# prip-lab/MSU-LatentAFIS

Hardware: AMD Instinct MI355X
Metric: latent queries/sec vs 100k rolled gallery (higher is better)
Workload: dtype f32

## Files before the change

msu-latentafis_amd/csrc/graph.hip:

```cpp
#include "afis_device.h"
#include <type_traits>
#include "atan2f_libm.h"
#include "graph_arith.h"
#include "stdsort_order.h"

namespace afis {

#define AFIS_PI 3.1415926
typedef unsigned long long u64;

#ifdef AFIS_PHASE_TIMING
__device__ u64 g_graph_phase[16];
#define GPH_INIT() u64 gph_t0 = __builtin_readcyclecounter()
#define GPH(i) do { if (threadIdx.x == 0) { const u64 t1_ = __builtin_readcyclecounter(); sm.ph[(i)] += t1_ - gph_t0; gph_t0 = t1_; } } while (0)
#define GPH_T0() const u64 gph_k0 = __builtin_readcyclecounter()
#define GPH_K(i) do { if (threadIdx.x == 0) sm.ph[(i)] += __builtin_readcyclecounter() - gph_k0; } while (0)
#define GPH_ZERO() do { if (threadIdx.x < 16) sm.ph[threadIdx.x] = 0; WSYNC(); } while (0)
#define GPH_FLUSH() do { WSYNC(); if (threadIdx.x < 16 && sm.ph[threadIdx.x]) atomicAdd(&g_graph_phase[threadIdx.x], sm.ph[threadIdx.x]); } while (0)
#else
#define GPH_INIT() do {} while (0)
#define GPH(i) do {} while (0)
#define GPH_T0() do {} while (0)
#define GPH_K(i) do {} while (0)
#define GPH_ZERO() do {} while (0)
// ... 103 lines not shown
template <class SM, int ref_tie>
__device__ __forceinline__ void sort_scores(SM& sm, int num, double thr)
{
    const int lane = threadIdx.x;
    constexpr int U = SM::U;
    uint32_t* const s_key = reinterpret_cast<uint32_t*>(sm.x.s.keys);
    uint32_t* const s_cnt = s_key + SM::N4;
    uint32_t* const s_gkey = reinterpret_cast<uint32_t*>(sm.y.cc);
    static_assert(sizeof(sm.x) >= (size_t)(SM::N4 + 128) * 4, "sort scratch exceeds the union");
    uint32_t m32[U]; int r[U];
    if (num <= 48) {
        const u64 mine = lane < num ? g_make_key(sm.b[lane], lane) : 0ull;
        if (lane < num) sm.x.s.keys[lane] = mine;
        WSYNC();
        int rr = 0;
        for (int k = 0; k < num; ++k) rr += sm.x.s.keys[k] > mine;
        if (ref_tie && num > 16) {
            int gg = 0;
            for (int k = 0; k < num; ++k) gg += (uint32_t)(sm.x.s.keys[k] >> 32) > (uint32_t)(mine >> 32);
            const bool tied = lane < num && gg != rr && !((double)sm.b[lane] < thr);
            if (__ballot(tied) != 0ull) {
                uint32_t* const k32 = reinterpret_cast<uint32_t*>(sm.x.s.keys) + 96;
                static_assert(sizeof(sm.x.s.keys) >= (96 + 48 + 48) * 4, "no room for the keys and the stack of the std::sort restatement");
                WSYNC();
                if (lane < num) { k32[lane] = (uint32_t)(mine >> 32); sm.y.os.order[lane] = (short)lane; }
                WSYNC();
                if (lane == 0) stdsort_prefix<uint16_t>(reinterpret_cast<uint16_t*>(sm.y.os.order), num, num, k32, reinterpret_cast<int*>(k32 + 48));
                WSYNC();
                return;
            }
        }
        WSYNC();
        if (lane < num) sm.y.os.order[rr] = (short)lane;
        WSYNC();
        return;
    }
    uint32_t kmin = 0xffffffffu, kmax = 0u;
#pragma unroll
    for (int u = 0; u < U; ++u) {
        const int t = lane + 64 * u;
        m32[u] = t < num ? g_ord_f32(sm.b[t]) : 0u;
        if (t < num) { s_key[t] = m32[u]; kmin = min(kmin, m32[u]); kmax = max(kmax, m32[u]); }
    }
#pragma unroll
    for (int off = 32; off >= 1; off >>= 1) { kmin = min(kmin, (uint32_t)__shfl_xor((int)kmin, off)); kmax = max(kmax, (uint32_t)__shfl_xor((int)kmax, off)); }
    const uint32_t span = kmax - kmin;
    const int sh = max(0, 26 - __clz((int)(span | 1u)));
    int bin[U];
#pragma unroll
    for (int u = 0; u < U; ++u) bin[u] = (int)((m32[u] - kmin) >> sh) & 63;
    s_cnt[lane] = 0u;
    WSYNC();
#pragma unroll
    for (int u = 0; u < U; ++u) if (lane + 64 * u < num) atomicAdd(&s_cnt[bin[u]], 1u);
    WSYNC();
    {
        const int own = (int)s_cnt[lane];
        int suf = own;
#pragma unroll
        for (int off = 1; off < 64; off <<= 1) { const int v = __shfl_down(suf, off); if (lane + off < 64) suf += v; }
        WSYNC();
        s_cnt[lane] = (uint32_t)(suf - own); s_cnt[64 + lane] = (uint32_t)(suf - own);
    }
    WSYNC();
#pragma unroll
    for (int u = 0; u < U; ++u) if (lane + 64 * u < num) s_gkey[atomicAdd(&s_cnt[bin[u]], 1u)] = m32[u];
    WSYNC();
    int rsum = 0;
#pragma unroll
    for (int u = 0; u < U; ++u) {
        r[u] = 0;
        if (lane + 64 * u < num) {
            const int lo = (int)s_cnt[64 + bin[u]], hi = (int)s_cnt[bin[u]];
            int c = lo;
            for (int k = lo; k < hi; ++k) c += s_gkey[k] > m32[u];
            r[u] = c; rsum += c;
        }
    }
    if (g_wave_sum(rsum) != num * (num - 1) / 2) {
        u64 mine[U];
        int gg[U];
#pragma unroll
        for (int u = 0; u < U; ++u) { const int t = lane + 64 * u; mine[u] = t < num ? ((u64)m32[u] << 32) | (uint32_t)(~(uint32_t)t) : 0ull; r[u] = 0; gg[u] = 0; }
        for (int k = 0; k < num; ++k) {
            const u64 kk = ((u64)s_key[k] << 32) | (uint32_t)(~(uint32_t)k);
#pragma unroll
            for (int u = 0; u < U; ++u) { r[u] += kk > mine[u]; gg[u] += s_key[k] > m32[u]; }
        }
        if (ref_tie) {
            bool tied = false;
#pragma unroll
            for (int u = 0; u < U; ++u) { const int t = lane + 64 * u; tied |= t < num && gg[u] != r[u] && !((double)sm.b[t] < thr); }
            if (__ballot(tied) != 0ull) {
                WSYNC();
#pragma unroll
                for (int u = 0; u < U; ++u) { const int t = lane + 64 * u; if (t < num) sm.y.os.order[t] = (short)t; }
                WSYNC();
                if (lane == 0) stdsort_prefix<uint16_t>(reinterpret_cast<uint16_t*>(sm.y.os.order), num, num, s_key, reinterpret_cast<int*>(s_cnt));
                WSYNC();
                return;
            }
        }
    }
    WSYNC();
#pragma unroll
    for (int u = 0; u < U; ++u) { const int t = lane + 64 * u; if (t < num) sm.y.os.order[r[u]] = (short)t; }
    WSYNC();
}

template <class SM, class Compat>
__device__ int greedy(SM& sm, int num, double thr, Compat compatible)
{
    const int lane = threadIdx.x;
    constexpr int U = SM::U;
    int idx[U], li[U], ri[U];
    bool alive[U];
#pragma unroll
    for (int u = 0; u < U; ++u) {
        const int p = lane + 64 * u;
        idx[u] = 0; li[u] = -1; ri[u] = -1; alive[u] = false;
        if (p < num) {
            idx[u] = sm.y.os.order[p];
            li[u] = l_row<SM>(sm.li[idx[u]]); ri[u] = r_pt<SM>(sm.ri[idx[u]]);
            alive[u] = !((double)sm.b[idx[u]] < thr);
        }
    }
    int nsel = 0;
    for (;;) {
        int first = -1, cidx = 0, cli = 0, cri = 0;
#pragma unroll
        for (int u = 0; u < U; ++u) {
            const u64 m = __ballot(alive[u]);
            if (first < 0 && m) {
                const int fl = __ffsll((long long)m) - 1;
                first = 64 * u + fl;
                cidx = __shfl(idx[u], fl); cli = __shfl(li[u], fl); cri = __shfl(ri[u], fl);
            }
        }
        if (first < 0) break;
        if (lane == 0) sm.y.os.sel[nsel] = (short)cidx;
        ++nsel;
#pragma unroll
        for (int u = 0; u < U; ++u) {
            if (alive[u]) {
                const int p = lane + 64 * u;
                if (p == first || li[u] == cli || ri[u] == cri || !compatible(cidx, idx[u])) alive[u] = false;
            }
        }
    }
    WSYNC();
    return nsel;
}

template <class SM>
__device__ void compact(SM& sm, int n)
{
    const int lane = threadIdx.x;
    float sim[SM::U]; short li[SM::U], ri[SM::U]; int2 xy[SM::U];
#pragma unroll
    for (int u = 0; u < SM::U; ++u) {
        const int t = lane + 64 * u;
        sim[u] = 0.0f;
        if (t < n) { const int s = sm.y.os.sel[t]; if constexpr (SM::OWN_SIM) sim[u] = sm.simv[s]; li[u] = sm.li[s]; ri[u] = sm.ri[s]; xy[u] = sm.xy[s]; }
    }
    WSYNC();
#pragma unroll
    for (int u = 0; u < SM::U; ++u) {
        const int t = lane + 64 * u;
        if (t < n) { if constexpr (SM::OWN_SIM) sm.simv[t] = sim[u]; sm.li[t] = li[u]; sm.ri[t] = ri[u]; sm.xy[t] = xy[u]; }
    }
    WSYNC();
}

template <class SM>
__device__ __forceinline__ float seq_sum(const SM& sm, int num)
{
    float sum = 0.0f;
    const float4* c4 = reinterpret_cast<const float4*>(sm.y.cc);
#pragma unroll 4
    for (int k = 0; k < (num + 3) / 4; ++k) { const float4 v = c4[k]; sum += v.x; sum += v.y; sum += v.z; sum += v.w; }
    return sum;
}

template <bool LOOKUP>
__device__ __forceinline__ bool pair_dist(const Pt& a, const Pt& o, const float* __restrict__ table, float& dist)
{
    float d1, d2; bool ok = true;
    if (LOOKUP) {
        const int dx1 = abs(a.lx - o.lx), dx2 = abs(a.rx - o.rx), dy1 = abs(a.ly - o.ly), dy2 = abs(a.ry - o.ry);
        ok = !((dx1 >= kDistN) | (dx2 >= kDistN) | (dy1 >= kDistN) | (dy2 >= kDistN));
        d1 = sqrt_rn_pos((float)(256 * (dx1 * dx1 + dy1 * dy1)));
        d2 = sqrt_rn_pos((float)(256 * (dx2 * dx2 + dy2 * dy2)));
        (void)table;
    } else {
        const float dx1 = (float)(a.lx - o.lx), dx2 = (float)(a.rx - o.rx), dy1 = (float)(a.ly - o.ly), dy2 = (float)(a.ry - o.ry);
        const float p = dx1 * dx1, q = dy1 * dy1, r = dx2 * dx2, s = dy2 * dy2;
        d1 = sqrt_rn_pos(p + q);
        d2 = sqrt_rn_pos(r + s);
    }
    dist = fabsf(d1 - d2);
    return ok;
}
template <bool LOOKUP>
__device__ __forceinline__ bool pair_compatible(const Pt& a, const Pt& o, const float* __restrict__ table)
{
    float s1, s2; bool ok = true;
    if (LOOKUP) {
        const int dx1 = abs(a.lx - o.lx), dx2 = abs(a.rx - o.rx), dy1 = abs(a.ly - o.ly), dy2 = abs(a.ry - o.ry);
        ok = !((dx1 >= kDistN) | (dx2 >= kDistN) | (dy1 >= kDistN) | (dy2 >= kDistN));
        s1 = (float)(256 * (dx1 * dx1 + dy1 * dy1)); s2 = (float)(256 * (dx2 * dx2 + dy2 * dy2));
    } else {
        const float dx1 = (float)(a.lx - o.lx), dx2 = (float)(a.rx - o.rx), dy1 = (float)(a.ly - o.ly), dy2 = (float)(a.ry - o.ry);
        const float p = dx1 * dx1, q = dy1 * dy1, r = dx2 * dx2, s = dy2 * dy2;
        s1 = p + q; s2 = r + s;
    }
    const float d1 = __builtin_amdgcn_sqrtf(s1), d2 = __builtin_amdgcn_sqrtf(s2);
    const float dist = fabsf(d1 - d2);
    const float slack = fmaxf(d1, d2) * 4.76837158e-7f;
    if (fabsf(dist - 30.0f) > slack) return ok && dist < 30.0f;
    float exact;
    pair_dist<LOOKUP>(a, o, table, exact);
    return ok && exact < 30.0f;
}
template <bool RANGE_TEST>
__device__ __forceinline__ bool tex_pair_dist(int2 a, int2 o, float& dist)
{
    float n1, n2;
    pair_n(a, o, n1, n2);
    dist = 16.0f * fabsf(sqrt_rn_int(n1) - sqrt_rn_int(n2));
    return RANGE_TEST ? tex_in_range(a, o) : true;
}
template <bool RANGE_TEST>
__device__ __forceinline__ bool tex_pair_compatible(int2 a, int2 o)
{
    float n1, n2;
    pair_n(a, o, n1, n2);
    const bool ok = RANGE_TEST ? tex_in_range(a, o) : true;
    return pair_compatible_n<true>(n1, n2) && ok;
}

__device__ __forceinline__ float minu_pair_dist(int2 a, int2 o)
{
    float n1, n2;
    pair_n(a, o, n1, n2);
    return fabsf(sqrt_rn_int(n1) - sqrt_rn_int(n2));
}
__device__ __forceinline__ bool minu_pair_compatible(int2 a, int2 o)
{
    float n1, n2;
    pair_n(a, o, n1, n2);
    return pair_compatible_n<false>(n1, n2);
}

__device__ __forceinline__ float h_of_x(float x)
{
    const float q0 = x * 0.04f;
    const float r = fmaf(-q0, 25.0f, x);
    const float h = fmaf(r, 0.04f, q0);
    return __builtin_amdgcn_fmed3f(h, 0.0f, 1.0f);
}
__device__ __forceinline__ float h_value(float dist)
{
    const float x = 30.0f - dist;
    const float q0 = x * 0.04f;
    const float r = fmaf(-q0, 25.0f, x);
    const float h = fmaf(r, 0.04f, q0);
    return __builtin_amdgcn_fmed3f(h, 0.0f, 1.0f);
}

template <class SM, bool LOOKUP, int ITERS, int MODE, int REF_TIE>
__device__ int dist_filter(SM& sm, int num, const float* __restrict__ table, const float* __restrict__ ext, SlabBuf slab)
{
    constexpr bool fast = MODE > 0;
    constexpr bool range_test = MODE == 1;
    auto compat_fast = [](int2 a, int2 o) -> bool { if (LOOKUP) return tex_pair_compatible<range_test>(a, o); return minu_pair_compatible(a, o); };
    auto dist_fast = [](int2 a, int2 o) -> float { float d; if (LOOKUP) { tex_pair_dist<range_test>(a, o, d); return d; } return minu_pair_dist(a, o); };
    constexpr int U = SM::U, W = SM::W, NMAX = SM::NMAX;
    [[maybe_unused]] constexpr int PH = LOOKUP ? 8 : 0;
    GPH_INIT();
    const int lane = threadIdx.x;
    for (int i = lane; i < num * W; i += 64) sm.hb[i / W][i % W] = 0u;
    int2 me[U];
#pragma unroll
    for (int u = 0; u < U; ++u) {
        const int t = lane + 64 * u;
        if (t < SM::N4) { sm.b[t] = t < num ? list_sim(sm, ext, t) : 0.0f; sm.y.cc[t] = 0.0f; }
        me[u] = t < num ? sm.xy[t] : make_int2(0, 0);
    }
    WSYNC();
    const int half = num >> 1;
    const bool even = !(num & 1);
    uint32_t* const hb0 = &sm.hb[0][0];
    auto pair = [&](int2 own, int t, int k, int2 other) {
        if (fast ? compat_fast(own, other) : pair_compatible<LOOKUP>(unpack_xy(own), unpack_xy(other), table)) {
            atomicOr(hb0 + (t * W + (k >> 5)), 1u << (k & 31));
            atomicOr(hb0 + (__umul24(k, W) + (t >> 5)), 1u << (t & 31));
        }
    };
    const int tail0 = num & ~63, R = num - tail0;
    const bool grouped = R > 0 && R <= 32;
    const int n_wide = grouped ? tail0 : num;
    uint32_t kb[U];
    const uint32_t num8 = (uint32_t)num * 8u;
#pragma unroll
    for (int u = 0; u < U; ++u) { const int t = lane + 64 * u; kb[u] = t < num ? (uint32_t)t * 8u : 0u; }
#ifndef AFIS_PAIR_UNROLL
// ... 59 lines not shown
    const int n_blk = (n_wide + 63) >> 6;
    if (n_blk >= U) pair_loop(std::integral_constant<int, U>{});
    else if (U > 1 && n_blk == U - 1) pair_loop(std::integral_constant<int, (U > 1 ? U - 1 : 1)>{});
    else if (n_blk > 0) pair_loop(std::integral_constant<int, U>{});
    if (grouped) {
        const int sh = R <= 8 ? 3 : R <= 16 ? 4 : 5, RG = 1 << sh, dstep = 64 >> sh;
        const int r = lane & (RG - 1), t = tail0 + r;
        const bool row = r < R;
        const int2 own = row ? sm.xy[t] : make_int2(0, 0);
        int d = 1 + (lane >> sh);
        int k = t + d; k = k >= num ? k - num : k;
        for (int d0 = 1; d0 <= half; d0 += dstep) {
            if (row && d <= half && !(d == half && even && t >= half)) pair(own, t, k, sm.xy[k]);
            d += dstep; k += dstep; k = k >= num ? k - num : k;
        }
    }
    WSYNC();
    GPH(PH + 0);
    int myrow[U], trip[U], rlen[U];
    const int Wn = (num + 31) / 32;
    {
        int cnt[U];
#pragma unroll
        for (int u = 0; u < U; ++u) {
            const int t = lane + 64 * u;
            int c = -1;
            if (t < num) {
                c = 0; for (int w = 0; w < Wn; ++w) c += __popc(sm.hb[t][w]);
                sm.y.os.sel[t] = (short)c;
                c = min(c >> 2, 15);
            }
            cnt[u] = c;
        }
        int base = 0;
        for (int bk = 15; bk >= 0; --bk) {
#pragma unroll
            for (int u = 0; u < U; ++u) {
                const bool in = cnt[u] == bk;
                const u64 m = __ballot(in);
                if (in) sm.y.os.order[base + g_lane_prefix(m)] = (short)(lane + 64 * u);
                base += __popcll(m);
            }
        }
        WSYNC();
#pragma unroll
        for (int u = 0; u < U; ++u) {
            const int p = lane + 64 * u;
            myrow[u] = p < num ? (int)sm.y.os.order[p] : -1;
            rlen[u] = myrow[u] >= 0 ? (int)sm.y.os.sel[myrow[u]] : 0;
            trip[u] = g_wave_max(rlen[u]);
        }
        WSYNC();
        for (int t = num + lane; t < SM::N4; t += 64) sm.y.cc[t] = 0.0f;
    }
    int2 mine[U];
#pragma unroll
    for (int u = 0; u < U; ++u) mine[u] = myrow[u] >= 0 ? sm.xy[myrow[u]] : make_int2(0, 0);
    constexpr bool kFlat = NMAX > 128;
    constexpr int kSlabN = kFlat ? kTexSlabSteps : kMinuSlabSteps;
    static_assert(kSlabN % 4 == 0, "the read loop takes blocks of four steps");
    static_assert((size_t)U * kSlabN * 64 * 5 == (kFlat ? kTexSlabWgBytes : kMinuSlabWgBytes), "slab layout and the size the host allocates differ");
    constexpr int kSlabBlk = kSlabN / 4;
    constexpr uint32_t kSlabIdx0 = (uint32_t)U * kSlabN * 64 * 4;
    const uint32_t lane16 = (uint32_t)lane * 16u, lane4 = (uint32_t)lane * 4u;
    auto put_block = [&](int e, const float (&h)[4], uint32_t k4) {
        __builtin_amdgcn_raw_buffer_store_b128(v4u{__float_as_uint(h[0]), __float_as_uint(h[1]), __float_as_uint(h[2]), __float_as_uint(h[3])}, slab, lane16, e * 1024, 0);
        __builtin_amdgcn_raw_buffer_store_b32(k4, slab, lane4, (int)kSlabIdx0 + e * 256, 0);
    };
    auto get_block = [&](int e, v4u& h, uint32_t& k4) {
        h = __builtin_amdgcn_raw_buffer_load_b128(slab, lane16, e * 1024, 0);
        k4 = __builtin_amdgcn_raw_buffer_load_b32(slab, lane4, (int)kSlabIdx0 + e * 256, 0);
    };
    int cur_w[U]; uint32_t cur_bits[U];
#pragma unroll
    for (int u = 0; u < U; ++u) { cur_w[u] = 0; cur_bits[u] = 0u; }
    auto value = [&](int2 own, int k) -> float {
        float dist;
        if (fast && LOOKUP) {
            float n1, n2;
            pair_n(own, sm.xy[k], n1, n2);
            return h_of_x(fmaf(-16.0f, fabsf(sqrt_rn_int(n1) - sqrt_rn_int(n2)), 30.0f));
        }
        if (fast) dist = dist_fast(own, sm.xy[k]);
        else pair_dist<LOOKUP>(unpack_xy(own), unpack_xy(sm.xy[k]), table, dist);
        return h_value(dist);
    };
    for (int it = 0; it < ITERS; ++it) {
#pragma unroll
        for (int u = 0; u < U; ++u) {
            const int t = myrow[u];
            const uint32_t* hrow = sm.hb[t >= 0 ? t : 0];
            float acc = 0.0f;
            if (it == 0) {
                if (t >= 0) {
                    int w = 0;
                    uint32_t bits = hrow[0];
                    for (int n0 = 0; n0 < trip[u]; n0 += 4) {
                        if (n0 == kSlabN) { cur_w[u] = w; cur_bits[u] = bits; }
                        float h4[4] = {0.0f, 0.0f, 0.0f, 0.0f};
                        uint32_t k4 = 0u;
#pragma unroll
                        for (int j = 0; j < 4; ++j) {
                            if (n0 + j < trip[u]) {
                                while (bits == 0u && w + 1 < Wn) { ++w; bits = hrow[w]; }
                                const bool have = bits != 0u;
                                const int k = (w * 32 + __ffs(bits) - 1) & 255;
                                bits &= bits - 1;
                                const float h = value(mine[u], k);
                                h4[j] = h; k4 |= (uint32_t)k << (8 * j);
                                const float p = h * sm.b[k];
                                acc += have ? p : 0.0f;
                            }
                        }
                        if (n0 < kSlabN) put_block(u * kSlabBlk + (n0 >> 2), h4, k4);
                    }
                }
            } else {
                const int nS = min(trip[u], kSlabN);
                v4u hc = {0u, 0u, 0u, 0u}; uint32_t kc = 0u;
                if (nS > 0) get_block(u * kSlabBlk, hc, kc);
                for (int n0 = 0; n0 < nS; n0 += 4) {
                    const float hn[4] = {__uint_as_float(hc.x), __uint_as_float(hc.y), __uint_as_float(hc.z), __uint_as_float(hc.w)};
                    const uint32_t kn = kc;
                    if (n0 + 4 < nS) get_block(u * kSlabBlk + (n0 >> 2) + 1, hc, kc);
#pragma unroll
                    for (int j = 0; j < 4; ++j) {
                        const float p = hn[j] * sm.b[(kn >> (8 * j)) & 255u];
                        acc += n0 + j < rlen[u] ? p : 0.0f;
                    }
                }
                if (trip[u] > kSlabN) {
                    int w = cur_w[u];
                    uint32_t bits = cur_bits[u];
                    for (int n = kSlabN; n < trip[u]; ++n) {
                        while (bits == 0u && w + 1 < Wn) { ++w; bits = t >= 0 ? hrow[w] : 0u; }
                        const bool have = bits != 0u;
                        const int k = (w * 32 + __ffs(bits) - 1) & 255;
                        bits &= bits - 1;
                        const float p = value(mine[u], k) * sm.b[k];
                        acc += have ? p : 0.0f;
                    }
                }
            }
            if (t >= 0) sm.y.cc[t] = acc;
        }
        WSYNC();
        const float sum = seq_sum(sm, num);
        const float scale = (float)(1.0 / ((double)sum + 0.00001));
#pragma unroll
        for (int u = 0; u < U; ++u) { const int t = lane + 64 * u; if (t < num) sm.b[t] = sm.y.cc[t] * scale; }
        WSYNC();
    }
    GPH(PH + 1);
    sort_scores<SM, REF_TIE>(sm, num, 0.0001);
    GPH(PH + 2);
    const int nsel = greedy(sm, num, 0.0001, [&sm, table, dist_fast](int a, int o) {
        if (!((sm.hb[a][o >> 5] >> (o & 31)) & 1u)) return false;
        float dist;
        if (fast) dist = dist_fast(sm.xy[a], sm.xy[o]);
        else pair_dist<LOOKUP>(unpack_xy(sm.xy[a]), unpack_xy(sm.xy[o]), table, dist);
        return !((double)h_value(dist) < 0.00001);
    });
    compact(sm, nsel);
    GPH(PH + 3);
    return nsel;
}

__device__ __forceinline__ float adjust_angle(float angle)
{
    if ((double)angle > AFIS_PI) angle = (float)((double)angle - 2 * AFIS_PI);
    else if ((double)angle < -AFIS_PI) angle = (float)((double)angle + 2 * AFIS_PI);
    return angle;
}
__device__ __forceinline__ float fold_pi(float d)
{
    if ((double)d > AFIS_PI) d = (float)(2 * AFIS_PI - (double)d);
    return d;
}
__device__ __forceinline__ float atan2_f32(float y, float x) { return afis_atan2f_libm(y, x); }

__device__ __forceinline__ bool angle_compatible(const Pt& p1, float lo1, float ro1, const Pt& p2, float lo2, float ro2)
{
    float angle_1 = adjust_angle(lo1 - lo2);
    float angle_2 = adjust_angle(ro1 - ro2);
    float angle_diff = fold_pi(fabsf(angle_1 - angle_2));
    if ((double)angle_diff > AFIS_PI / 4.) return false;
    const float dx_1 = (float)(p1.lx - p2.lx), dy_1 = (float)(p1.ly - p2.ly);
    const float line_angle_1 = -atan2_f32(dy_1, dx_1);
    angle_1 = adjust_angle(lo1 - line_angle_1);
    const float dx_2 = (float)(p1.rx - p2.rx), dy_2 = (float)(p1.ry - p2.ry);
    const float line_angle_2 = -atan2_f32(dy_2, dx_2);
    angle_2 = adjust_angle(ro1 - line_angle_2);
    angle_diff = fold_pi(fabsf(angle_1 - angle_2));
    if ((double)angle_diff > AFIS_PI / 6.) return false;
    angle_1 = adjust_angle(lo2 - line_angle_1);
    angle_2 = adjust_angle(ro2 - line_angle_2);
    angle_diff = fold_pi(fabsf(angle_1 - angle_2));
    if ((double)angle_diff > AFIS_PI / 6.) return false;
    return true;
}

template <class SM, int REF_TIE>
__device__ int angle_filter(SM& sm, int num, const float* __restrict__ lori, const float* __restrict__ rori)
{
    constexpr int W = SM::W;
    [[maybe_unused]] constexpr int PH = SM::NMAX > 128 ? 8 : 0;
    GPH_INIT();
    const int lane = threadIdx.x;
    if constexpr (SM::ALIAS_ORI) {
        for (int t = lane; t < num; t += 64) { sm.b[t] = lori[l_row<SM>(sm.li[t])]; sm.y.cc[t] = rori[r_pt<SM>(sm.ri[t])]; }
        for (int i = lane; i < num * W; i += 64) sm.hb[i / W][i % W] = 0u;
    } else {
        for (int t = lane; t < num; t += 64) { sm.x.s.lo[t] = lori[l_row<SM>(sm.li[t])]; sm.x.s.ro[t] = rori[r_pt<SM>(sm.ri[t])]; }
        for (int i = lane; i < num * W; i += 64) sm.hb[i / W][i % W] = 0u;
        const float s0 = (float)(1.0 / num);
        for (int t = lane; t < SM::N4; t += 64) { sm.b[t] = t < num ? s0 : 0.0f; sm.y.cc[t] = 0.0f; }
    }
    WSYNC();
    const int half = num >> 1;
    const bool even = !(num & 1);
    auto pair = [&](int t, int k) {
        const int i = t < k ? t : k, j = t < k ? k : t;
        bool ok;
        if constexpr (SM::ALIAS_ORI) ok = angle_compatible(unpack_xy(sm.xy[i]), sm.b[i], sm.y.cc[i], unpack_xy(sm.xy[j]), sm.b[j], sm.y.cc[j]);
        else ok = angle_compatible(unpack_xy(sm.xy[i]), sm.x.s.lo[i], sm.x.s.ro[i], unpack_xy(sm.xy[j]), sm.x.s.lo[j], sm.x.s.ro[j]);
        if (ok) {
            atomicOr(&sm.hb[i][j >> 5], 1u << (j & 31));
            atomicOr(&sm.hb[j][i >> 5], 1u << (i & 31));
        }
    };
    const int tail0 = num & ~63, R = num - tail0;
    const bool grouped = R > 0 && R <= 32;
    const int n_wide = grouped ? tail0 : num;
    for (int d = 1; n_wide > 0 && d <= half; ++d) {
        for (int t = lane; t < n_wide; t += 64) {
            if (d == half && even && t >= half) continue;
            int k = t + d; if (k >= num) k -= num;
            pair(t, k);
        }
    }
    if (grouped) {
        const int sh = R <= 8 ? 3 : R <= 16 ? 4 : 5, RG = 1 << sh, dstep = 64 >> sh;
        const int r = lane & (RG - 1), t = tail0 + r;
        int d = 1 + (lane >> sh);
        int k = t + d; k = k >= num ? k - num : k;
        for (int d0 = 1; d0 <= half; d0 += dstep) {
            if (r < R && d <= half && !(d == half && even && t >= half)) pair(t, k);
            d += dstep; k += dstep; k = k >= num ? k - num : k;
        }
    }
    WSYNC();
    if constexpr (SM::ALIAS_ORI) {
        const float s0 = (float)(1.0 / num);
        for (int t = lane; t < SM::N4; t += 64) { sm.b[t] = t < num ? s0 : 0.0f; sm.y.cc[t] = 0.0f; }
        WSYNC();
    }
    GPH(PH + 4);
    for (int it = 0; it < 5; ++it) {
        for (int t = lane; t < num; t += 64) {
            float s1 = 0.0f;
            for (int w = 0; w < (num + 31) / 32; ++w) {
                uint32_t bits = sm.hb[t][w];
                while (bits) { const int k = w * 32 + __ffs(bits) - 1; bits &= bits - 1; s1 += sm.b[k]; }
            }
            sm.y.cc[t] = s1;
        }
        WSYNC();
        float sum = seq_sum(sm, num);
        sum = (float)(1.0 / ((double)sum + 0.00001));
        for (int t = lane; t < num; t += 64) sm.b[t] = sm.y.cc[t] * sum;
        WSYNC();
    }
    GPH(PH + 5);
    sort_scores<SM, REF_TIE>(sm, num, 0.001);
    const int nsel = greedy(sm, num, 0.001, [&sm](int a, int o) { return (sm.hb[a][o >> 5] >> (o & 31)) & 1u; });
    compact(sm, nsel);
    GPH(PH + 6);
    return nsel;
}

template <class SM, bool LOOKUP, int ITERS, int REF_TIE>
__device__ __forceinline__ float graph_score(SM& sm, int num, const float* __restrict__ table, const float* __restrict__ lori,
                                             const float* __restrict__ rori, const float* __restrict__ ext, SlabBuf slab, int& n_survivors, int stop_after = 2, int mode = 0)
{
    n_survivors = num;
    if (stop_after == 0) return 0.0f;
    if (mode == 2 && LOOKUP) num = dist_filter<SM, LOOKUP, ITERS, 2, REF_TIE>(sm, num, table, ext, slab);
    else if (mode >= 1) num = dist_filter<SM, LOOKUP, ITERS, 1, REF_TIE>(sm, num, table, ext, slab);
    else num = dist_filter<SM, LOOKUP, ITERS, 0, REF_TIE>(sm, num, table, ext, slab);
    n_survivors = num;
    if (mode >= 1) {
        for (int t = threadIdx.x; t < num; t += 64) {
            const int2 v = sm.xy[t];
            int lx, ly, rx, ry;
            unpack_h2(v.x, lx, ly); unpack_h2(v.y, rx, ry);
            sm.xy[t] = pack_xy(lx, ly, rx, ry);
        }
        WSYNC();
    }
    if (stop_after == 1) return 0.0f;
    n_survivors = 0;
    if (num < 2) return 0.0f;
    num = angle_filter<SM, REF_TIE>(sm, num, lori, rori);
    n_survivors = num;
    for (int t = threadIdx.x; t < num; t += 64) sm.b[t] = list_sim(sm, ext, t);
    WSYNC();
    float score = 0.0f;
    for (int i = 0; i < num; ++i) score += sm.b[i];
    return score;
}

struct GraphTap { MinuCand* out; int32_t* n; int stage; };
template <class SM>
__device__ __forceinline__ void tap_write(const GraphTap& tap, const SM& sm, const float* __restrict__ ext, long long task, int n, int cap)
{
    for (int t = threadIdx.x; t < n; t += 64) { MinuCand c; c.sim = list_sim(sm, ext, t); c.li = l_row<SM>(sm.li[t]); c.ri = r_pt<SM>(sm.ri[t]); tap.out[(size_t)task * cap + t] = c; }
    if (threadIdx.x == 0) tap.n[task] = n;
}

#ifndef AFIS_TEX_WAVES
#define AFIS_TEX_WAVES 4
#endif
typedef WaveSmem<kTopTex, false> TexSmem;
constexpr int kTexRegs = (kTexMax + 63) / 64;
constexpr int kTexFast = 256;
constexpr int kTexFastRegs = kTexFast / 64;

template <int REF_TIE>
__global__ __launch_bounds__(64) __attribute__((amdgpu_waves_per_eu(AFIS_TEX_WAVES, AFIS_TEX_WAVES))) void k_graph_texture(QueryDev q, GalleryDev g, const float* __restrict__ table_dist,
                                                      const float* __restrict__ rm_val, const int32_t* __restrict__ rm_arg,
                                                      const float* __restrict__ rm_cv, const int32_t* __restrict__ rm_n,
                                                      float* __restrict__ parts, unsigned char* slab_all, GraphTap tap)
{
    __shared__ TexSmem sm;
    const SlabBuf slab = g_slab_buf(slab_all + (size_t)blockIdx.x * kTexSlabWgBytes, (uint32_t)kTexSlabWgBytes);
    const int lane = threadIdx.x;
    GPH_ZERO();
    const int n_tasks = q.nq * g.G;
    for (;;) {
        const int task = next_task(g.task_ctr + 0);
        if (task >= n_tasks) break;
        GPH_T0();
        const int qi = task / g.G, gi = task - qi * g.G;
        const int l0 = q.lt_off[qi], n_lt = q.lt_off[qi + 1] - l0;
        const int r0 = g.tex_off[gi], n_rt = g.tex_off[gi + 1] - r0;
        float* out = parts + (size_t)task * 4 + 3;
        if (n_lt <= 0 || n_rt <= 0) { if (lane == 0) { *out = 0.0f; if (tap.out) tap.n[task] = -1; } continue; }
        const size_t o = (size_t)task * q.lt_pad;
        int num;
        if (n_lt > kTopTex) {
            const bool compact = rm_n != nullptr;
            const int n_in = compact ? rm_n[task] : n_lt;
            if (compact && n_in >= kTopTex && n_in <= kTexFast) {
                uint32_t key[kTexFastRegs]; int arg[kTexFastRegs];
                uint32_t kmin = 0xffffffffu, kmax = 0u;
#pragma unroll
                for (int u = 0; u < kTexFastRegs; ++u) {
                    const int e = u * 64 + lane;
                    const bool in = e < n_in;
                    key[u] = in ? g_ord_f32(rm_cv[o + e]) : 0u;
                    arg[u] = in ? rm_arg[o + e] : 0;
                    kmax = max(kmax, key[u]);
                    if (in) kmin = min(kmin, key[u]);
                }
                kmin = g_wave_min_u32(kmin); kmax = g_wave_max_u32(kmax);
                const int shift = max(0, 27 - __clz((int)((kmax - kmin) >> 1) | 1));
                uint32_t* const s_cnt = reinterpret_cast<uint32_t*>(sm.b);
                uint32_t* const s_gkey = sm.x.sortbuf;
                static_assert(TexSmem::N4 >= 128 && sizeof(sm.x.sortbuf) >= (size_t)kTexFast * 4, "the counting arrays of the compact S7 exceed their buffers");
                int bin[kTexFastRegs], r[kTexFastRegs];
#pragma unroll
                for (int u = 0; u < kTexFastRegs; ++u) bin[u] = min((int)((key[u] - kmin) >> shift), 63);
                s_cnt[lane] = 0u;
                WSYNC();
#pragma unroll
                for (int u = 0; u < kTexFastRegs; ++u) if (u * 64 + lane < n_in) atomicAdd(&s_cnt[bin[u]], 1u);
                WSYNC();
                {
                    const int own = (int)s_cnt[lane];
                    int suf = own;
#pragma unroll
                    for (int off = 1; off < 64; off <<= 1) { const int v = __shfl_down(suf, off); if (lane + off < 64) suf += v; }
                    WSYNC();
                    s_cnt[lane] = (uint32_t)(suf - own); s_cnt[64 + lane] = (uint32_t)(suf - own);
                }
                WSYNC();
#pragma unroll
                for (int u = 0; u < kTexFastRegs; ++u) if (u * 64 + lane < n_in) s_gkey[atomicAdd(&s_cnt[bin[u]], 1u)] = key[u];
                WSYNC();
                int rsum = 0;
#pragma unroll
                for (int u = 0; u < kTexFastRegs; ++u) {
                    r[u] = 0;
                    if (u * 64 + lane < n_in) {
                        const int lo = (int)s_cnt[64 + bin[u]], hi = (int)s_cnt[bin[u]];
                        int c = lo;
                        for (int k = lo; k < hi; ++k) c += s_gkey[k] > key[u];
                        r[u] = c; rsum += c;
                    }
                }
                if (g_wave_sum(rsum) != n_in * (n_in - 1) / 2) {
                    WSYNC();
#pragma unroll
                    for (int u = 0; u < kTexFastRegs; ++u) if (u * 64 + lane < n_in) s_gkey[u * 64 + lane] = key[u];
                    WSYNC();
                    u64 mine[kTexFastRegs];
#pragma unroll
                    for (int u = 0; u < kTexFastRegs; ++u) { mine[u] = ((u64)key[u] << 32) | (uint32_t)(~(uint32_t)(u * 64 + lane)); r[u] = 0; }
                    for (int k = 0; k < n_in; ++k) {
                        const u64 kk = ((u64)s_gkey[k] << 32) | (uint32_t)(~(uint32_t)k);
#pragma unroll
                        for (int u = 0; u < kTexFastRegs; ++u) r[u] += kk > mine[u];
                    }
                }
#pragma unroll
                for (int u = 0; u < kTexFastRegs; ++u) {
                    const int e = u * 64 + lane;
                    if (e < n_in && r[u] < kTopTex) { sm.li[r[u]] = tex_pack_l(arg[u] & 0xffff, e); sm.ri[r[u]] = tex_pack_r(arg[u] >> 16, e); }
                }
                num = kTopTex;
            } else {
                const int n_regs = (n_in + 63) >> 6;
                uint32_t key[kTexRegs]; int arg[kTexRegs];
#pragma unroll
                for (int u = 0; u < kTexRegs; ++u) {
                    const int e = u * 64 + lane;
                    const bool in = e < n_in;
                    key[u] = 0u; arg[u] = 0;
                    if (u < n_regs) {
                        key[u] = in ? g_ord_f32(compact ? rm_cv[o + e] : rm_val[o + e]) : 0u;
                        arg[u] = in ? rm_arg[o + e] : 0;
                    }
                }
                uint32_t T = 0;
                for (int bit = 31; bit >= 0; --bit) {
                    const uint32_t cand = T | (1u << bit);
                    int c = 0;
#pragma unroll
                    for (int u = 0; u < kTexRegs; ++u) if (u < n_regs) c += g_wave_popc(key[u] >= cand);
                    if (c >= kTopTex) { T = cand; if (c == kTopTex) break; }
                }
                int n_gt = 0;
#pragma unroll
                for (int u = 0; u < kTexRegs; ++u) if (u < n_regs) n_gt += g_wave_popc(key[u] > T);
                const int need = kTopTex - n_gt;
                int base_gt = 0, base_eq = 0;
                uint32_t* const key32 = sm.x.pick.keys;
#pragma unroll
                for (int u = 0; u < kTexRegs; ++u) {
                    if (u < n_regs) {
                        const int e = u * 64 + lane;
                        const bool gt = key[u] > T, eq = key[u] == T;
                        const u64 mg = __ballot(gt), me = __ballot(eq);
                        int pos = -1;
                        if (gt) pos = base_gt + g_lane_prefix(mg);
                        else if (eq) { const int r = base_eq + g_lane_prefix(me); if (r < need) pos = n_gt + r; }
                        if (pos >= 0) { key32[pos] = key[u]; sm.x.pick.te[pos] = tex_pack_l(compact ? arg[u] & 0xffff : e, e); sm.x.pick.targ[pos] = tex_pack_r(compact ? arg[u] >> 16 : arg[u], e); }
                        base_gt += __popcll(mg); base_eq += __popcll(me);
                    }
                }
                WSYNC();
                num = kTopTex;
                uint32_t m32[TexSmem::U]; int r[TexSmem::U];
                uint32_t* const s_cnt = reinterpret_cast<uint32_t*>(sm.b);
                uint32_t* const s_gkey = reinterpret_cast<uint32_t*>(sm.y.cc);
                int dmax = 0;
#pragma unroll
                for (int u = 0; u < TexSmem::U; ++u) {
                    const int t = lane + 64 * u;
                    m32[u] = t < num ? key32[t] : T;
                    dmax = max(dmax, (int)((m32[u] - T) >> 1));
                }
                dmax = g_wave_max(dmax);
                const int shift = max(0, 27 - __clz(dmax | 1));
                int bin[TexSmem::U];
#pragma unroll
                for (int u = 0; u < TexSmem::U; ++u) bin[u] = min((int)((m32[u] - T) >> shift), 63);
                s_cnt[lane] = 0u;
                WSYNC();
#pragma unroll
                for (int u = 0; u < TexSmem::U; ++u) if (lane + 64 * u < num) atomicAdd(&s_cnt[bin[u]], 1u);
                WSYNC();
                {
                    const int own = (int)s_cnt[lane];
                    int suf = own;
#pragma unroll
                    for (int off = 1; off < 64; off <<= 1) { const int v = __shfl_down(suf, off); if (lane + off < 64) suf += v; }
                    WSYNC();
                    s_cnt[lane] = (uint32_t)(suf - own); s_cnt[64 + lane] = (uint32_t)(suf - own);
                }
                WSYNC();
#pragma unroll
                for (int u = 0; u < TexSmem::U; ++u) if (lane + 64 * u < num) s_gkey[atomicAdd(&s_cnt[bin[u]], 1u)] = m32[u];
                WSYNC();
#pragma unroll
                for (int u = 0; u < TexSmem::U; ++u) {
                    r[u] = 0;
                    if (lane + 64 * u < num) {
                        const int lo = (int)s_cnt[64 + bin[u]], hi = (int)s_cnt[bin[u]];
                        int c = lo;
                        for (int k = lo; k < hi; ++k) c += s_gkey[k] > m32[u];
                        r[u] = c;
                    }
                }
                int rsum = 0;
#pragma unroll
                for (int u = 0; u < TexSmem::U; ++u) rsum += r[u];
                if (g_wave_sum(rsum) != kTopTex * (kTopTex - 1) / 2) {
                    u64 mine[TexSmem::U];
#pragma unroll
                    for (int u = 0; u < TexSmem::U; ++u) { const int t = lane + 64 * u; mine[u] = t < num ? ((u64)key32[t] << 32) | (uint32_t)(~(uint32_t)(sm.x.pick.te[t] & 1023)) : 0ull; r[u] = 0; }
                    for (int k = 0; k < num; ++k) {
                        const u64 kk = ((u64)key32[k] << 32) | (uint32_t)(~(uint32_t)(sm.x.pick.te[k] & 1023));
#pragma unroll
                        for (int u = 0; u < TexSmem::U; ++u) r[u] += kk > mine[u];
                    }
                }
#pragma unroll
                for (int u = 0; u < TexSmem::U; ++u) {
                    const int t = lane + 64 * u;
                    if (t < num) { sm.li[r[u]] = sm.x.pick.te[t]; sm.ri[r[u]] = sm.x.pick.targ[t]; }
                }
            }
        } else {
            num = n_lt;
            for (int t = lane; t < num; t += 64) { sm.li[t] = tex_pack_l(t, t); sm.ri[t] = tex_pack_r(rm_n ? rm_arg[o + t] >> 16 : rm_arg[o + t], t); }
        }
        WSYNC();
        int out_of_range = 0, not_small = 0;
        short2 lp4[TexSmem::U], rp4[TexSmem::U];
#pragma unroll
        for (int u = 0; u < TexSmem::U; ++u) {
            const int t = lane + 64 * u;
            lp4[u] = make_short2(0, 0); rp4[u] = make_short2(0, 0);
            if (t < num) {
                lp4[u] = q.lt_xy[l0 + (sm.li[t] & 1023)]; rp4[u] = g.tex_xy[r0 + (sm.ri[t] & 1023)];
                out_of_range |= (lp4[u].x | lp4[u].y | rp4[u].x | rp4[u].y) & ~2047;
                not_small |= ((unsigned)lp4[u].x > 49u) | ((unsigned)lp4[u].y > 49u) | ((unsigned)rp4[u].x > 49u) | ((unsigned)rp4[u].y > 49u);
            }
        }
        const int mode = __ballot(out_of_range != 0) != 0ull ? 0 : (__ballot(not_small != 0) == 0ull ? 2 : 1);
#pragma unroll
        for (int u = 0; u < TexSmem::U; ++u) {
            const int t = lane + 64 * u;
            if (t < num) sm.xy[t] = mode ? make_int2(pack_h2(lp4[u].x, lp4[u].y), pack_h2(rp4[u].x, rp4[u].y)) : pack_xy(lp4[u].x, lp4[u].y, rp4[u].x, rp4[u].y);
        }
        WSYNC();
        GPH_K(15);
        int n_surv;
        const float* const row_max = (rm_n ? rm_cv : rm_val) + o;
        const float score = graph_score<TexSmem, true, 3, REF_TIE>(sm, num, table_dist, q.lt_ori + l0, g.tex_ori + r0, row_max, slab, n_surv, tap.out ? tap.stage : 2, mode);
        if (lane == 0) *out = score;
        if (tap.out) tap_write(tap, sm, row_max, task, n_surv, kTopTex);
        WSYNC();
    }
    GPH_FLUSH();
}

hipError_t launch_graph_texture(const QueryDev& q, const GalleryDev& g, const float* table_dist,
                                const float* rm_val, const int32_t* rm_arg, const float* rm_cv, const int32_t* rm_n, float* parts, void* slab, size_t slab_bytes, MinuCand* tap_out, int32_t* tap_n, int tap_stage, hipStream_t stream)
{
    const long long n_tasks = (long long)q.nq * g.G;
    if (n_tasks <= 0) return hipSuccess;
    if (n_tasks > 0x7ffffff0LL || !g.task_ctr) return hipErrorInvalidValue;
    const int grid = graph_texture_grid(n_tasks);
    if (!slab || slab_bytes < (size_t)grid * kTexSlabWgBytes) return hipErrorInvalidValue;
    hipError_t e0 = hipMemsetAsync(g.task_ctr + 0, 0, 4, stream);
    if (e0 != hipSuccess) return e0;
    const GraphTap tap{tap_out, tap_n, tap_stage & 255};
    if ((tap_stage >> 8) & 1) hipLaunchKernelGGL(k_graph_texture<1>, dim3(grid), dim3(64), 0, stream, q, g, table_dist, rm_val, rm_arg, rm_cv, rm_n, parts, (unsigned char*)slab, tap);
    else hipLaunchKernelGGL(k_graph_texture<0>, dim3(grid), dim3(64), 0, stream, q, g, table_dist, rm_val, rm_arg, rm_cv, rm_n, parts, (unsigned char*)slab, tap);
    return hipGetLastError();
}

typedef WaveSmem<kTopMinu, true> MinuGraphSmem;

#ifndef AFIS_MINU_WAVES
#define AFIS_MINU_WAVES 6
#endif
template <int REF_TIE>
__global__ __launch_bounds__(64) __attribute__((amdgpu_waves_per_eu(AFIS_MINU_WAVES, AFIS_MINU_WAVES))) void k_graph_minutiae(QueryDev q, GalleryDev g, const MinuCand* __restrict__ cands,
                                                       const int32_t* __restrict__ cand_n, float* __restrict__ parts,
                                                       short4* __restrict__ corr_out, int32_t* __restrict__ corr_n, unsigned char* slab_all, GraphTap tap)
{
    __shared__ MinuGraphSmem sm;
    const SlabBuf slab = g_slab_buf(slab_all + (size_t)blockIdx.x * kMinuSlabWgBytes, (uint32_t)kMinuSlabWgBytes);
    const int lane = threadIdx.x;
    GPH_ZERO();
    const int n_tasks = q.nq * 3 * g.G;
    for (;;) {
        const int task = next_task(g.task_ctr + 1);
        if (task >= n_tasks) break;
        GPH_T0();
        const int gi = task % g.G;
        const int qs = task / g.G;
        const int qi = qs / 3, s = qs - qi * 3;
        float* out = parts + ((size_t)qi * g.G + gi) * 4 + s;
        const int num = cand_n[task];
        if (num <= 0) { if (lane == 0) { *out = 0.0f; if (corr_n) corr_n[task] = 0; if (tap.out) tap.n[task] = -1; } continue; }
        const int l0 = q.lm_off[qs], r0 = g.minu_off[gi];
        const MinuCand* c = cands + (size_t)task * kTopMinu;
        int out_of_range = 0;
        short2 lp2[MinuGraphSmem::U], rp2[MinuGraphSmem::U];
#pragma unroll
        for (int u = 0; u < MinuGraphSmem::U; ++u) {
            const int t = lane + 64 * u;
            lp2[u] = make_short2(0, 0); rp2[u] = make_short2(0, 0);
            if (t < num) {
                const MinuCand cd = c[t];
                sm.simv[t] = cd.sim; sm.li[t] = cd.li; sm.ri[t] = cd.ri;
                lp2[u] = q.lm_xy[l0 + cd.li]; rp2[u] = g.minu_xy[r0 + cd.ri];
                out_of_range |= (lp2[u].x | lp2[u].y | rp2[u].x | rp2[u].y) & ~2047;
            }
        }
        const int mode = __ballot(out_of_range != 0) == 0ull ? 1 : 0;
#pragma unroll
        for (int u = 0; u < MinuGraphSmem::U; ++u) {
            const int t = lane + 64 * u;
            if (t < num) sm.xy[t] = mode ? make_int2(pack_h2(lp2[u].x, lp2[u].y), pack_h2(rp2[u].x, rp2[u].y)) : pack_xy(lp2[u].x, lp2[u].y, rp2[u].x, rp2[u].y);
        }
        WSYNC();
        GPH_K(7);
        int n_surv;
        const float score = graph_score<MinuGraphSmem, false, 5, REF_TIE>(sm, num, nullptr, q.lm_ori + l0, g.minu_ori + r0, nullptr, slab, n_surv, tap.out ? tap.stage : 2, mode);
        if (lane == 0) *out = score;
        if (tap.out) tap_write(tap, sm, nullptr, task, n_surv, kTopMinu);
        if (corr_out) {
            for (int t = lane; t < n_surv; t += 64) {
                const Pt p = unpack_xy(sm.xy[t]);
                corr_out[(size_t)task * kTopMinu + t] = make_short4((short)p.lx, (short)p.ly, (short)p.rx, (short)p.ry);
            }
            if (lane == 0) corr_n[task] = n_surv;
        }
        WSYNC();
    }
    GPH_FLUSH();
}

hipError_t launch_graph_minutiae(const QueryDev& q, const GalleryDev& g, const MinuCand* cands, const int32_t* cand_n,
                                 float* parts, short4* corr_out, int32_t* corr_n, void* slab, size_t slab_bytes, MinuCand* tap_out, int32_t* tap_n, int tap_stage, hipStream_t stream, bool join)
{
    const long long n_tasks = (long long)q.nq * 3 * g.G;
    if (n_tasks <= 0) return hipSuccess;
    if (n_tasks > 0x7ffffff0LL || !g.task_ctr) return hipErrorInvalidValue;
    const int grid = graph_minutiae_grid(n_tasks);
    if (!slab || slab_bytes < (size_t)grid * kMinuSlabWgBytes) return hipErrorInvalidValue;
    hipError_t e0 = join ? hipSuccess : hipMemsetAsync(g.task_ctr + 1, 0, 4, stream);
    if (e0 != hipSuccess) return e0;
    const GraphTap tap{tap_out, tap_n, tap_stage & 255};
    if ((tap_stage >> 8) & 1) hipLaunchKernelGGL(k_graph_minutiae<1>, dim3(grid), dim3(64), 0, stream, q, g, cands, cand_n, parts, corr_out, corr_n, (unsigned char*)slab, tap);
    else hipLaunchKernelGGL(k_graph_minutiae<0>, dim3(grid), dim3(64), 0, stream, q, g, cands, cand_n, parts, corr_out, corr_n, (unsigned char*)slab, tap);
    return hipGetLastError();
}

__global__ __launch_bounds__(256) void k_debug_atan2_grid(int R, float* __restrict__ out)
{
    const int W = 2 * R + 1;
    const long long idx = (long long)blockIdx.x * 256 + threadIdx.x;
    if (idx >= (long long)W * W) return;
    const int dy = (int)(idx / W) - R, dx = (int)(idx % W) - R;
    out[idx] = atan2_f32((float)dy, (float)dx);
}
hipError_t launch_debug_atan2_grid(int R, float* out, hipStream_t stream)
{
    const long long n = (long long)(2 * R + 1) * (2 * R + 1);
    hipLaunchKernelGGL(k_debug_atan2_grid, dim3((unsigned)((n + 255) / 256)), dim3(256), 0, stream, R, out);
    return hipGetLastError();
}

__device__ __forceinline__ void arith_check(bool tex, float f1, float f2, unsigned long long* cnt)
{
    const float d = fabsf(sqrt_rn_pos(f1) - sqrt_rn_pos(f2));
    const bool ref = tex ? 16.0f * d < 30.0f : d < 30.0f;
    const int a = tex ? pair_compatible_alg<true>(f1, f2) : pair_compatible_alg<false>(f1, f2);
    const bool full = tex ? pair_compatible_n<true>(f1, f2) : pair_compatible_n<false>(f1, f2);
    atomicAdd(cnt + 0, 1ull);
    if (a == 2) atomicAdd(cnt + 1, 1ull);
    if ((a != 2 && (a == 1) != ref) || full != ref) atomicAdd(cnt + 2, 1ull);
}
__global__ __launch_bounds__(256) void k_debug_graph_arith(int part, unsigned long long* __restrict__ cnt)
{
    constexpr unsigned kMaxN = 2u * 2047u * 2047u;
    if (part == 0) {
        const unsigned n = blockIdx.x * 256u + threadIdx.x;
        if (n <= kMaxN && __float_as_uint(sqrt_rn_int((float)n)) != __float_as_uint(sqrt_rn_pos((float)n))) atomicAdd(cnt, 1ull);
    } else if (part == 3) {
        const int dx = (int)blockIdx.x - 2047, dy = (int)(blockIdx.y * 256u + threadIdx.x) - 2047;
        if (dy > 2047) return;
        const int ax = dx > 0 ? dx : 0, ox = dx > 0 ? 0 : -dx, ay = dy > 0 ? dy : 0, oy = dy > 0 ? 0 : -dy;
        const float n = diff_n(pack_h2(ax, ay), pack_h2(ox, oy));
        int bx, by; unpack_h2(pack_h2(ax, ay), bx, by);
        if (__float_as_uint(n) != __float_as_uint((float)(dx * dx + dy * dy)) || bx != ax || by != ay) atomicAdd(cnt, 1ull);
    } else if (part == 1) {
        const unsigned n1 = blockIdx.x, n2 = blockIdx.y * 256u + threadIdx.x;
        if (n1 <= 4802u && n2 <= 4802u) arith_check(true, (float)n1, (float)n2, cnt + 1);
    } else {
        const unsigned n1 = blockIdx.x * 256u + threadIdx.x;
        if (n1 > kMaxN) return;
        const double a = sqrt((double)n1);
        for (int sg = -1; sg <= 1; sg += 2) {
            const double b = a + 30.0 * sg;
            if (b < 0) continue;
            const long long c = (long long)(b * b + 0.5);
            for (int j = -12; j <= 12; ++j) { const long long n2 = c + j; if (n2 >= 0 && n2 <= (long long)kMaxN) arith_check(false, (float)n1, (float)n2, cnt + 4); }
        }
    }
}
hipError_t launch_debug_graph_arith(unsigned long long* cnt8, hipStream_t stream)
{
    constexpr unsigned kMaxN = 2u * 2047u * 2047u;
    hipError_t e = hipMemsetAsync(cnt8, 0, 64, stream);
    if (e != hipSuccess) return e;
    hipLaunchKernelGGL(k_debug_graph_arith, dim3((kMaxN + 256) / 256), dim3(256), 0, stream, 0, cnt8);
    hipLaunchKernelGGL(k_debug_graph_arith, dim3(4803, 19), dim3(256), 0, stream, 1, cnt8);
    hipLaunchKernelGGL(k_debug_graph_arith, dim3((kMaxN + 256) / 256), dim3(256), 0, stream, 2, cnt8);
    hipLaunchKernelGGL(k_debug_graph_arith, dim3(4095, 16), dim3(256), 0, stream, 3, cnt8 + 7);
    return hipGetLastError();
}

hipError_t read_graph_phase_cycles(unsigned long long* out16, bool reset)
{
#ifdef AFIS_PHASE_TIMING
    hipError_t e = hipMemcpyFromSymbol(out16, HIP_SYMBOL(g_graph_phase), 16 * sizeof(u64));
    if (e != hipSuccess) return e;
    if (reset) { u64 z[16] = {}; e = hipMemcpyToSymbol(HIP_SYMBOL(g_graph_phase), z, sizeof(z)); }
    return e;
#else
    for (int i = 0; i < 16; ++i) out16[i] = 0;
    return hipSuccess;
#endif
}

}
```

Measured before the change: 53.65.

## Skip score sort with bounded greedy max-selection and register-resident small angle filter

Replaces the full sort-then-greedy selection with a bounded number of wave-wide argmax rounds over register-held keys. It falls back to the sort path only when candidates remain after the round cap. Adds a specialised angle filter for up to 32 candidates that builds the compatibility matrix as per-lane bitmasks and runs the power iteration via readlane, avoiding LDS bitmap traffic and syncs. Ties are broken by lowest index, which may differ from the reference tie order, so the fast path is enabled only when REF_TIE==0.

```diff
diff --git a/msu-latentafis_amd/csrc/graph.hip b/msu-latentafis_amd/csrc/graph.hip
--- a/msu-latentafis_amd/csrc/graph.hip
+++ b/msu-latentafis_amd/csrc/graph.hip
@@ -279,6 +279,72 @@
     return nsel;
 }
 
+__device__ __forceinline__ int g_opaque_lane() { int l = threadIdx.x; asm volatile("" : "+v"(l)); return l; }
+
+#ifndef AFIS_SEL_ROUNDS
+#define AFIS_SEL_ROUNDS 16
+#endif
+constexpr int kSelRounds = AFIS_SEL_ROUNDS;
+template <class SM, int U, class Compat>
+__device__ __forceinline__ int select_greedy(SM& sm, int num, int max_rounds, const uint32_t (&key)[U], const int (&li)[U], const int (&ri)[U], bool (&alive)[U], Compat compatible)
+{
+    const int lane = g_opaque_lane();
+    int nsel = 0;
+    const int rounds = min(num, max_rounds);
+    for (int round = 0; round < rounds; ++round) {
+        bool any = false;
+        uint32_t best = 0u;
+#pragma unroll
+        for (int u = 0; u < U; ++u) { any |= alive[u]; best = max(best, alive[u] ? key[u] : 0u); }
+        if (__ballot(any) == 0ull) break;
+        best = g_wave_max_u32(best);
+        int cidx = -1, cli = 0, cri = 0;
+#pragma unroll
+        for (int u = 0; u < U; ++u) {
+            const u64 m = __ballot(alive[u] && key[u] == best);
+            if (cidx < 0 && m) {
+                const int fl = __ffsll((long long)m) - 1;
+                cidx = 64 * u + fl;
+                cli = __shfl(li[u], fl); cri = __shfl(ri[u], fl);
+            }
+        }
+        if (lane == 0) sm.y.os.sel[nsel] = (short)cidx;
+        ++nsel;
+#pragma unroll
+        for (int u = 0; u < U; ++u) {
+            if (alive[u]) {
+                const int t = lane + 64 * u;
+                if (t == cidx || li[u] == cli || ri[u] == cri || !compatible(cidx, t)) alive[u] = false;
+            }
+        }
+    }
+    bool left = false;
+#pragma unroll
+    for (int u = 0; u < U; ++u) left |= alive[u];
+    if (__ballot(left) != 0ull) return -1;
+    WSYNC();
+    return nsel;
+}
+template <class SM, class Compat>
+__device__ __forceinline__ int select_greedy_lds(SM& sm, int num, double thr, Compat compatible)
+{
+    const int lane = g_opaque_lane();
+    constexpr int U = SM::U;
+    uint32_t key[U]; int li[U], ri[U]; bool alive[U];
+#pragma unroll
+    for (int u = 0; u < U; ++u) {
+        const int t = lane + 64 * u;
+        key[u] = 0u; li[u] = -1; ri[u] = -1; alive[u] = false;
+        if (t < num) {
+            const float v = sm.b[t];
+            key[u] = g_ord_f32(v);
+            li[u] = l_row<SM>(sm.li[t]); ri[u] = r_pt<SM>(sm.ri[t]);
+            alive[u] = !((double)v < thr);
+        }
+    }
+    return select_greedy<SM, U>(sm, num, kSelRounds, key, li, ri, alive, compatible);
+}
+
 template <class SM>
 __device__ void compact(SM& sm, int n)
 {
@@ -644,15 +710,20 @@
         WSYNC();
     }
     GPH(PH + 1);
-    sort_scores<SM, REF_TIE>(sm, num, 0.0001);
-    GPH(PH + 2);
-    const int nsel = greedy(sm, num, 0.0001, [&sm, table, dist_fast](int a, int o) {
+    auto compatible = [&sm, table, dist_fast](int a, int o) {
         if (!((sm.hb[a][o >> 5] >> (o & 31)) & 1u)) return false;
         float dist;
         if (fast) dist = dist_fast(sm.xy[a], sm.xy[o]);
         else pair_dist<LOOKUP>(unpack_xy(sm.xy[a]), unpack_xy(sm.xy[o]), table, dist);
         return !((double)h_value(dist) < 0.00001);
-    });
+    };
+    int nsel = -1;
+    if constexpr (REF_TIE == 0) nsel = select_greedy_lds(sm, num, 0.0001, compatible);
+    GPH(PH + 2);
+    if (nsel < 0) {
+        sort_scores<SM, REF_TIE>(sm, num, 0.0001);
+        nsel = greedy(sm, num, 0.0001, compatible);
+    }
     compact(sm, nsel);
     GPH(PH + 3);
     return nsel;
@@ -692,9 +763,77 @@
     return true;
 }
 
+#ifndef AFIS_ANGLE_SMALL
+#define AFIS_ANGLE_SMALL 32
+#endif
+constexpr int kAngleSmall = AFIS_ANGLE_SMALL;
+template <class SM>
+__device__ int angle_filter_small(SM& sm, int num, const float* __restrict__ lori, const float* __restrict__ rori)
+{
+    static_assert(kAngleSmall <= 32, "a row of H is one 32-bit mask");
+    [[maybe_unused]] constexpr int PH = SM::NMAX > 128 ? 8 : 0;
+    GPH_INIT();
+    const int lane = g_opaque_lane();
+    const bool in = lane < num;
+    const int myli = l_row<SM>(sm.li[in ? lane : 0]), myri = r_pt<SM>(sm.ri[in ? lane : 0]);
+    float* s_lo; float* s_ro;
+    if constexpr (SM::ALIAS_ORI) { s_lo = sm.b; s_ro = sm.y.cc; } else { s_lo = sm.x.s.lo; s_ro = sm.x.s.ro; }
+    if (in) { s_lo[lane] = lori[myli]; s_ro[lane] = rori[myri]; }
+    WSYNC();
+    const int half = num >> 1;
+    const bool even = !(num & 1);
+    const int sh = num <= 8 ? 3 : num <= 16 ? 4 : 5, RG = 1 << sh, dstep = 64 >> sh;
+    const int r = lane & (RG - 1);
+    const bool row = r < num;
+    const int t = row ? r : 0;
+    const int2 own_xy = sm.xy[t];
+    const float own_lo = s_lo[t], own_ro = s_ro[t];
+    uint32_t A = 0u;
+    int d = 1 + (lane >> sh);
+    int k = t + d; k = k >= num ? k - num : k;
+    for (int d0 = 1; d0 <= half; d0 += dstep) {
+        if (row && d <= half && !(d == half && even && t >= half)) {
+            const int2 o_xy = sm.xy[k];
+            const float o_lo = s_lo[k], o_ro = s_ro[k];
+            const bool low = t < k;
+            const int2 xy1 = low ? own_xy : o_xy, xy2 = low ? o_xy : own_xy;
+            if (angle_compatible(unpack_xy(xy1), low ? own_lo : o_lo, low ? own_ro : o_ro, unpack_xy(xy2), low ? o_lo : own_lo, low ? o_ro : own_ro)) A |= 1u << k;
+        }
+        d += dstep; k += dstep; k = k >= num ? k - num : k;
+    }
+    A |= (uint32_t)__shfl_xor((int)A, 32);
+    if (sh <= 4) A |= (uint32_t)__shfl_xor((int)A, 16);
+    if (sh <= 3) A |= (uint32_t)__shfl_xor((int)A, 8);
+    uint32_t H = A;
+    for (int kk = 0; kk < num; ++kk) H |= (((uint32_t)__builtin_amdgcn_readlane((int)A, kk) >> (lane & 31)) & 1u) << kk;
+    if (!in) H = 0u;
+    GPH(PH + 4);
+    float bv = in ? (float)(1.0 / num) : 0.0f;
+    for (int it = 0; it < 5; ++it) {
+        float s1 = 0.0f;
+        for (int kk = 0; kk < num; ++kk) {
+            const float bk = __uint_as_float((uint32_t)__builtin_amdgcn_readlane((int)__float_as_uint(bv), kk));
+            s1 += (H >> kk) & 1u ? bk : 0.0f;
+        }
+        float sum = 0.0f;
+        for (int kk = 0; kk < num; ++kk) sum += __uint_as_float((uint32_t)__builtin_amdgcn_readlane((int)__float_as_uint(s1), kk));
+        sum = (float)(1.0 / ((double)sum + 0.00001));
+        bv = s1 * sum;
+    }
+    GPH(PH + 5);
+    const uint32_t key[1] = {g_ord_f32(bv)};
+    const int li[1] = {in ? myli : -1}, ri[1] = {in ? myri : -1};
+    bool alive[1] = {in && !((double)bv < 0.001)};
+    const int nsel = select_greedy<SM, 1>(sm, num, num, key, li, ri, alive, [H](int a, int) { return (H >> a) & 1u; });
+    compact(sm, nsel);
+    GPH(PH + 6);
+    return nsel;
+}
+
 template <class SM, int REF_TIE>
 __device__ int angle_filter(SM& sm, int num, const float* __restrict__ lori, const float* __restrict__ rori)
 {
+    if constexpr (REF_TIE == 0) { if (num <= kAngleSmall) return angle_filter_small(sm, num, lori, rori); }
     constexpr int W = SM::W;
     [[maybe_unused]] constexpr int PH = SM::NMAX > 128 ? 8 : 0;
     GPH_INIT();
@@ -764,8 +903,13 @@
         WSYNC();
     }
     GPH(PH + 5);
-    sort_scores<SM, REF_TIE>(sm, num, 0.001);
-    const int nsel = greedy(sm, num, 0.001, [&sm](int a, int o) { return (sm.hb[a][o >> 5] >> (o & 31)) & 1u; });
+    auto compatible = [&sm](int a, int o) { return (sm.hb[a][o >> 5] >> (o & 31)) & 1u; };
+    int nsel = -1;
+    if constexpr (REF_TIE == 0) nsel = select_greedy_lds(sm, num, 0.001, compatible);
+    if (nsel < 0) {
+        sort_scores<SM, REF_TIE>(sm, num, 0.001);
+        nsel = greedy(sm, num, 0.001, compatible);
+    }
     compact(sm, nsel);
     GPH(PH + 6);
     return nsel;
@@ -795,7 +939,7 @@
     if (num < 2) return 0.0f;
     num = angle_filter<SM, REF_TIE>(sm, num, lori, rori);
     n_survivors = num;
-    for (int t = threadIdx.x; t < num; t += 64) sm.b[t] = list_sim(sm, ext, t);
+    for (int t = REF_TIE == 0 ? g_opaque_lane() : (int)threadIdx.x; t < num; t += 64) sm.b[t] = list_sim(sm, ext, t);
     WSYNC();
     float score = 0.0f;
     for (int i = 0; i < num; ++i) score += sm.b[i];
@@ -804,9 +948,9 @@
 
 struct GraphTap { MinuCand* out; int32_t* n; int stage; };
 template <class SM>
-__device__ __forceinline__ void tap_write(const GraphTap& tap, const SM& sm, const float* __restrict__ ext, long long task, int n, int cap)
-{
-    for (int t = threadIdx.x; t < n; t += 64) { MinuCand c; c.sim = list_sim(sm, ext, t); c.li = l_row<SM>(sm.li[t]); c.ri = r_pt<SM>(sm.ri[t]); tap.out[(size_t)task * cap + t] = c; }
+__device__ __forceinline__ void tap_write(const GraphTap& tap, const SM& sm, const float* __restrict__ ext, long long task, int n, int cap, int lane)
+{
+    for (int t = lane; t < n; t += 64) { MinuCand c; c.sim = list_sim(sm, ext, t); c.li = l_row<SM>(sm.li[t]); c.ri = r_pt<SM>(sm.ri[t]); tap.out[(size_t)task * cap + t] = c; }
     if (threadIdx.x == 0) tap.n[task] = n;
 }
 
@@ -1043,7 +1187,7 @@
         const float* const row_max = (rm_n ? rm_cv : rm_val) + o;
         const float score = graph_score<TexSmem, true, 3, REF_TIE>(sm, num, table_dist, q.lt_ori + l0, g.tex_ori + r0, row_max, slab, n_surv, tap.out ? tap.stage : 2, mode);
         if (lane == 0) *out = score;
-        if (tap.out) tap_write(tap, sm, row_max, task, n_surv, kTopTex);
+        if (tap.out) tap_write(tap, sm, row_max, task, n_surv, kTopTex, REF_TIE == 0 ? g_opaque_lane() : lane);
         WSYNC();
     }
     GPH_FLUSH();
@@ -1116,7 +1260,7 @@
         int n_surv;
         const float score = graph_score<MinuGraphSmem, false, 5, REF_TIE>(sm, num, nullptr, q.lm_ori + l0, g.minu_ori + r0, nullptr, slab, n_surv, tap.out ? tap.stage : 2, mode);
         if (lane == 0) *out = score;
-        if (tap.out) tap_write(tap, sm, nullptr, task, n_surv, kTopMinu);
+        if (tap.out) tap_write(tap, sm, nullptr, task, n_surv, kTopMinu, REF_TIE == 0 ? g_opaque_lane() : lane);
         if (corr_out) {
             for (int t = lane; t < n_surv; t += 64) {
                 const Pt p = unpack_xy(sm.xy[t]);
```

Measured after the change: 53.87, median of 6. Within noise of the previous version (+0.4%).
